# cvxopt/smcp

Measured on AMD Instinct MI355X. Metric: Newton KKT solves/sec, higher is better.
Workload: dtype f64; 1 GPU; synth50k nested block-arrow SDP n=50000, 8073 cliques, m=100; kktsolver=chol, n=50000, cliques=8073, m=100, blkval_doubles=2493568, update_doubles=10689536, parallelism=single

## Files before the change

### smcp_amd/csrc/capi.hip

```cpp
#include <hip/hip_runtime.h>
#include <memory>
#include <unordered_map>

#include <algorithm>
#include <chrono>
#include <cstdio>
#include <cstring>
#include <map>
#include <new>
#include <atomic>
#include <thread>
#include <type_traits>
#include <vector>

#include "../../include/smcp_amd.h"
#include "constraints.hpp"
#include "context.hpp"
#include "hostpar.hpp"
#include "switches.hpp"
#include "front_generic.hip"
#include "front_mfma.hip"
#include "front_large.hip"
#include "front_top.hip"
#include "front_inv.hip"
#include "front_n16.hip"
#include "front_downfam.hip"
#include "front_fam.hip"
#include "front_upfam.hip"
#include "front_fam2.hip"
#include "front_lfsp.hip"
#include "front_leafgram.hip"
#include "front_famt.hip"
#include "front_flow.hip"
#include "front_mrc.hip"
#include "front_edm.hip"
#include "front_psd.hip"
#include "front_trmm.hip"
#include "front_syr2k.hip"
#include "front_symm.hip"

using namespace smcp;

#define HIPCHK(x)                                                                        \
  do {                                                                                   \
    hipError_t e_ = (x);                                                                 \
    if (e_ != hipSuccess) {                                                              \
      fprintf(stderr, "smcp_amd: HIP error %s at %s:%d\n", hipGetErrorString(e_), __FILE__, __LINE__); \
      return SMCP_EHIP;                                                                  \
    }                                                                                    \
  } while (0)

namespace {

enum {
  KID_chol_level = 0, KID_llt_level, KID_pinv_level, KID_gather_level, KID_completion_all,
  KID_hess_up_level, KID_hess_down_level, KID_hess_down_inv_all, KID_hess_up_inv_level, KID_scale_an,
  KID_factor_yaa, KID_trsm_fwd_level, KID_trsm_bwd_level, KID_amap, KID_aadj, KID_scatter_constraints,
  KID_dense_potrf, KID_dense_potrs, KID_vec_axpby, KID_axpby, KID_reduce_cliques, KID_reduce_final,
  KID_hess_up_mfma, KID_hess_down_mfma, KID_chol_mfma, KID_pinv_mfma, KID_prep_lk,
  KID_hess_up_mfma_hbm, KID_hess_down_mfma_hbm, KID_chol_mfma_hbm, KID_pinv_mfma_hbm,
  KID_gram_partial, KID_gram_reduce, KID_hess_up_pad,
  KID_lf_assemble, KID_lf_clear_upd, KID_lf_up1, KID_lf_up2, KID_lf_up3, KID_lf_down1, KID_lf_down2, KID_lf_down3,
  KID_lf_pinv1, KID_lf_pinv2, KID_lf_diag, KID_lf_chol_panel, KID_lf_chol_trail, KID_lf_pack_upd,
  KID_lf_prep_s, KID_lf_prep_row, KID_lf_prep_k, KID_factor_yaa_lds,
  KID_factor_inverse, KID_hess_down_inv_mfma, KID_hess_down_inv_mfma_hbm, KID_hess_up_inv_mfma, KID_hess_up_inv_mfma_hbm,
  KID_completion_mfma, KID_completion_mfma_hbm, KID_lf_copy_an, KID_lf_ri_an, KID_lf_dinv1, KID_lf_dinv2,
  KID_lf_uinv1, KID_lf_uinv2, KID_lf_completion, KID_hess_up_n16, KID_llt_mfma, KID_llt_mfma_hbm, KID_lf_llt,
  KID_hess_up_fam, KID_qr_rmul, KID_qr_dots, KID_qr_comb, KID_qr_small, KID_fam2_prep, KID_mid_chol, KID_lf_diag_inv, KID_lfsp_up, KID_lfsp_prep, KID_leaf_gram, KID_leaf_tables, KID_fam_sparse, KID_gram_diag128, KID_lf_assemble_lds, KID_fam_terms, KID_famt_prep, KID_lf_assemble_lds_dyn, KID_lf_zsp, KID_fam_terms_grp, KID_lf_assemble_fz, KID_factor_inverse_lds, KID_chol_flow,
  KID_mrc_diag, KID_mrc_rank, KID_mrc_reduce, KID_mrc_factor, KID_cut_signs, KID_cut_weights,
  KID_edm_rank, KID_edm_reduce, KID_edm_factor, KID_edm_dense, KID_hess_down_fam, KID_hess_up_fam1,
  KID_psd_zero, KID_psd_scatter, KID_psd_solve, KID_psd_fill, KID_top_chol, KID_lf_trtri,
  KID_trmm_n, KID_trmm_t, KID_trmm_mm, KID_trmm_combine, KID_syr2k_fma, KID_syr2k_mm,
  KID_symm_fma, KID_symm_mm, KID_symm_combine,
  KID_potrs_many_small, KID_potrs_many_step, KID_aadj_sub_many, KID_kkt_many_y, KID_kkt_many_scale,
  KID_qr_dots_many, KID_qr_many_sum, KID_qr_many_small, KID_qr_many_mid, KID_qr_comb_many,
  KID_res_inv_table, KID_res_combine, KID_res_y, KID_res_norms, KID_kkt_many_sub,
  KID_COUNT
};
const char* const KID_NAMES[KID_COUNT] = {
  "k_chol_level", "k_llt_level", "k_pinv_level", "k_gather_level", "k_completion_all",
  "k_hess_up_level", "k_hess_down_level", "k_hess_down_inv_all", "k_hess_up_inv_level", "k_scale_an",
  "k_factor_yaa", "k_trsm_fwd_level", "k_trsm_bwd_level", "k_amap", "k_aadj", "k_scatter_constraints",
  "k_dense_potrf", "k_dense_potrs", "k_vec_axpby", "k_axpby", "k_reduce_cliques", "k_reduce_final",
  "k_hess_up_mfma<true>", "k_hess_down_mfma<true>", "k_chol_mfma<true>", "k_pinv_mfma<true>", "k_prep_lk",
  "k_hess_up_mfma<false>", "k_hess_down_mfma<false>", "k_chol_mfma<false>", "k_pinv_mfma<false>",
  "k_gram_partial", "k_gram_reduce", "k_hess_up_pad",
  "k_lf_assemble", "k_lf_clear_upd", "k_lf_up1", "k_lf_up2", "k_lf_up3", "k_lf_down1", "k_lf_down2", "k_lf_down3",
  "k_lf_pinv1", "k_lf_pinv2", "k_lf_diag", "k_lf_chol_panel", "k_lf_chol_trail", "k_lf_pack_upd",
  "k_lf_prep_s", "k_lf_prep_row", "k_lf_prep_k", "k_factor_yaa_lds",
  "k_factor_inverse", "k_hess_down_inv_mfma<true>", "k_hess_down_inv_mfma<false>", "k_hess_up_inv_mfma<true>",
  "k_hess_up_inv_mfma<false>", "k_completion_mfma<true>", "k_completion_mfma<false>", "k_lf_copy_an", "k_lf_ri_an",
  "k_lf_dinv1", "k_lf_dinv2", "k_lf_uinv1", "k_lf_uinv2", "k_lf_completion", "k_hess_up_n16",
  "k_llt_mfma<true>", "k_llt_mfma<false>", "k_lf_llt", "k_hess_up_fam",
  "k_stack_trsm", "k_stack_dots", "k_stack_comb", "k_qr_small", "k_fam2_prep", "k_mid_chol", "k_lf_diag_inv", "k_lfsp_up", "k_lfsp_prep", "k_leaf_pairs", "k_leaf_tables", "k_fam_sparse", "k_gram_diag128", "k_lf_assemble_lds", "k_fam_terms", "k_famt_prep", "k_lf_assemble_lds_dyn", "k_lf_zsp", "k_fam_terms_grp", "k_lf_assemble_fz", "k_factor_inverse_lds", "k_chol_flow",
  "k_mrc_diag", "k_mrc_rank", "k_mrc_reduce", "k_mrc_factor", "k_cut_signs", "k_cut_weights",
  "k_edm_rank", "k_edm_reduce", "k_edm_factor", "k_edm_dense", "k_hess_down_fam", "k_hess_up_fam1",
  "k_psd_zero", "k_psd_scatter", "k_psd_solve", "k_psd_fill", "k_top_chol", "k_lf_trtri",
  "k_trmm_n", "k_trmm_t", "k_trmm_mm", "k_trmm_combine", "k_syr2k_fma", "k_syr2k_mm",
  "k_symm_fma", "k_symm_mm", "k_symm_combine",
  "k_potrs_many_small", "k_potrs_many_step", "k_aadj_sub_many", "k_kkt_many_y", "k_kkt_many_scale",
  "k_stack_dots_many", "k_qr_many_sum", "k_qr_many_small", "k_qr_many_mid", "k_stack_comb_many",
  "k_res_inv_table", "k_res_combine", "k_res_y", "k_res_norms", "k_kkt_many_sub"};

inline void note_launch(csp_ctx* c, int kid) {
  const hipError_t e = hipGetLastError();
  if (e != hipSuccess && !c->launch_err) {
    c->launch_err = (int)e;
    fprintf(stderr, "smcp_amd: launch of %s failed: %s\n", (kid >= 0 && kid < KID_COUNT) ? KID_NAMES[kid] : "?", hipGetErrorString(e));
  }
}
inline hipError_t end_call(csp_ctx* c) {
  hipError_t e = hipGetLastError();
  if (e == hipSuccess && c->launch_err) e = c->launch_err > 0 ? (hipError_t)c->launch_err : hipErrorLaunchFailure;
  c->launch_err = 0;
  return e;
}

__global__ void k_race_spin(long long ticks) {
  const long long t0 = wall_clock64();
  for (int it = 0; it < (1 << 22) && wall_clock64() - t0 < ticks; ++it) __builtin_amdgcn_s_sleep(8);
}
struct RaceInject {
  std::atomic<uint64_t> state{0};
  std::atomic<int64_t> injected{0};
  std::atomic<int> max_us{200};
  std::atomic<int> drop_joins{0};
  bool on() const { return state.load(std::memory_order_relaxed) != 0; }
  void seed(uint64_t s) { state.store(s ? (s * 0x9E3779B97F4A7C15ull) | 1ull : 0ull); }
  uint64_t next() {
    uint64_t x = state.load(std::memory_order_relaxed);
    x ^= x << 13; x ^= x >> 7; x ^= x << 17;
    state.store(x | 1ull, std::memory_order_relaxed);
    return x;
  }
};
// ... 1725 lines not shown
      f.resize(S.nsn, 0);
      return put64(f);
    }
    case CSP_Q_MRC_CLAMPED:
      if (out) out[0] = c->mrc_clamped;
      return 1;
    case CSP_Q_EDM_CLAMPED:
      if (out) out[0] = c->edm_clamped;
      return 1;
  }
  return SMCP_EINVAL;
}

int csp_maxcardsearch(int64_t n, const int64_t* colptr, const int64_t* rowind, int64_t* order) {
  if (n <= 0 || !colptr || !rowind || !order) return SMCP_EINVAL;
  maxcardsearch(n, colptr, rowind, order);
  return 0;
}
int csp_mindegree(int64_t n, const int64_t* colptr, const int64_t* rowind, int64_t* order) {
  if (n <= 0 || !colptr || !rowind || !order) return SMCP_EINVAL;
  mindegree(n, colptr, rowind, order);
  return 0;
}
int csp_index_map(const csp_ctx* c, int64_t cnt, const int64_t* I, const int64_t* J, int64_t* out) {
  if (!c || cnt < 0) return SMCP_EINVAL;
  index_map(c->S, cnt, I, J, out);
  return 0;
}

}

#include "setup.hip"

extern "C" {

int64_t csp_device_bytes(const csp_ctx* c) { return c ? c->D.mem.total : 0; }

static int cholesky_impl(csp_ctx* c, double* x, void* stream, int set, bool li_last = false);
int csp_cholesky(csp_ctx* c, double* x, void* stream) { return cholesky_impl(c, x, stream, 0); }
int csp_cholesky_part(csp_ctx* c, double* x, int set, void* stream) {
  if (set < 1 || set > 2 || !c || !c->sets[set].lev2 || use_generic(c)) return SMCP_EINVAL;
  return cholesky_impl(c, x, stream, set);
}
static int cholesky_impl(csp_ctx* c, double* x, void* stream, int set, bool li_last) {
  if (int rc = ready(c)) return rc;
  invalidate_tags(c, x);
  hipStream_t st = (hipStream_t)stream;
  TreeArgs a = tree_args(c);
  HIPCHK(zero_flag(c, st));
  if (!use_generic(c)) {
    MfmaArgs a0 = mfma_args(c, nullptr, 0, 1);
    a0.LK = nullptr;
    for (int64_t l = 0; l < c->S.nlev; ++l)
      for_level_classes(c, l, a0, [&](bool lds, MfmaArgs am, int cnt, size_t bytes, int thr) {
        if (lds) launch_lds(c, KID_chol_mfma, k_chol_mfma<true>, dim3(cnt), dim3(fact_threads(am, thr, 0)),
                            (size_t)mfma_lds_doubles_for(WK_CHOL, am.nnmax, am.namax) * sizeof(double), st, am, x, (double*)nullptr);
        else if (use_large() && c->D.gp_tptr) lf_chol(c, am, cnt, x, st, li_last && l == c->S.nlev - 1);
        else launch_lds(c, KID_chol_mfma_hbm, k_chol_mfma<false>, dim3(cnt), dim3(thr), 0, st, am, x, (double*)nullptr);
      }, set);
  } else
  for_levels_up(c, [&](const int32_t* lev, int cnt) {
    a.lev = lev;
    launch(c, KID_chol_level, k_chol_level, dim3(cnt), dim3(NT), st, a, x);
  });
  HIPCHK(end_call(c));
  return fetch_info(c, st);
}

int csp_llt(csp_ctx* c, double* x, void* stream) {
  if (int rc = ready(c)) return rc;
  invalidate_tags(c, x);
  hipStream_t st = (hipStream_t)stream;
  TreeArgs a = tree_args(c);
  if (!use_generic(c)) {
    MfmaArgs a0 = mfma_args(c, nullptr, 0, 1);
    a0.LK = nullptr;
    dim3 blk(256);
    for (int64_t l = 0; l < c->S.nlev; ++l)
      for_level_classes(c, l, a0, [&](bool lds, MfmaArgs am, int cnt, size_t bytes, int thr) {
        if (lds) launch_lds(c, KID_llt_mfma, k_llt_mfma<true>, dim3(cnt), dim3(thr), bytes, st, am, x);
        else if (use_large()) {
          const int mtA = tiles64(am.namax), ntN = tiles64(am.nnmax);
          const int ntile = ntN * (ntN + 1) / 2 + mtA * ntN + mtA * (mtA + 1) / 2;
          launch(c, KID_lf_llt, k_lf_llt, dim3(umax1(ntile), cnt), blk, st, am, x, 0);
          launch(c, KID_lf_llt, k_lf_llt, dim3(umax1(ntile), cnt), blk, st, am, x, 1);
          lf_assemble(c, am, cnt, 1, x, 0, 2, st);
          if (am.namax) launch(c, KID_lf_pack_upd, k_lf_pack_upd, dim3(umax1(std::min(64, (am.namax * am.namax + 255) / 256)), cnt), blk, st, am);
        } else launch_lds(c, KID_llt_mfma_hbm, k_llt_mfma<false>, dim3(cnt), dim3(thr), 0, st, am, x);
      });
  } else
  for_levels_up(c, [&](const int32_t* lev, int cnt) {
    a.lev = lev;
    launch(c, KID_llt_level, k_llt_level, dim3(cnt), dim3(NT), st, a, x);
  });
  HIPCHK(end_call(c));
  return 0;
}

static int projected_inverse_impl(csp_ctx* c, double* x, void* stream, int set, bool have_li = false);
int csp_projected_inverse(csp_ctx* c, double* x, void* stream) { return projected_inverse_impl(c, x, stream, 0); }
int csp_projected_inverse_part(csp_ctx* c, double* x, int set, void* stream) {
  if (set < 1 || set > 2 || !c || !c->sets[set].lev2 || use_generic(c)) return SMCP_EINVAL;
  return projected_inverse_impl(c, x, stream, set);
}
static int projected_inverse_impl(csp_ctx* c, double* x, void* stream, int set, bool have_li) {
  if (int rc = ready(c)) return rc;
  invalidate_tags(c, x);
  hipStream_t st = (hipStream_t)stream;
  TreeArgs a = tree_args(c);
  if (!use_generic(c)) {
    if (set) { prep_lk_set(c, set, x, st); c->D.lk_tag_L = nullptr; c->D.lk_tag_Y = nullptr; }
    else {
    prep_lk(c, x, st, have_li);
    c->D.lk_tag_L = nullptr;
    c->D.lk_tag_Y = x;
    }
    const bool whole = !set;
    MfmaArgs a0 = mfma_args(c, nullptr, 0, 1);
    const bool keep_yaa = !set && !cache_off() && c->D.yaa && c->S.updlen() > 0;
    if (keep_yaa) a0.t.upd = c->D.yaa;
    for (int64_t l = c->S.nlev - 1; l >= 0; --l)
      for_level_classes(c, l, a0, [&](bool lds, MfmaArgs am, int cnt, size_t bytes, int thr) {
        if (lds) launch_lds(c, KID_pinv_mfma, k_pinv_mfma<true>, dim3(cnt), dim3(fact_threads(am, thr, 1)),
                            (size_t)mfma_lds_doubles_for(WK_PINV, am.nnmax, am.namax) * sizeof(double), st, am, x);
        else if (use_large()) lf_pinv(c, am, cnt, x, st);
        else launch_lds(c, KID_pinv_mfma_hbm, k_pinv_mfma<false>, dim3(cnt), dim3(thr), 0, st, am, x);
      }, set);
    if (keep_yaa) {
      c->D.yaa_tag = x;
      c->D.fac_tag = c->D.faci_tag = nullptr;
      c->D.part_valid = false;
      fp_record(c, 2, x, st);
    }
    if (whole) fp_record(c, 1, x, st);
  } else
  for_levels_down(c, [&](const int32_t* lev, int cnt) {
    a.lev = lev;
    launch(c, KID_pinv_level, k_pinv_level, dim3(cnt), dim3(NT), st, a, x);
  });
  HIPCHK(end_call(c));
  return 0;
}

constexpr int SCALING_FAC = 1;
static bool leafgram_ok(csp_ctx* c, int64_t mcols);
static bool scaling_overlap_on() {
  static int on = -1;
  if (on < 0) { const char* e = sw_str("SMCP_SCALING_OVERLAP"); on = (e && e[0] == '0') ? 0 : 1; }
  return on == 1;
}
static int scaling_impl(csp_ctx* c, double* L, double* Y, int flags, hipStream_t st) {
  DeviceCtx& D = c->D;
  const Symbolic& S = c->S;
  const int64_t bl = S.blklen();
  if (c->scal_lstar < 0) {
    int64_t ls = S.nlev;
    while (ls > 0 && c->lvl[(size_t)ls - 1].nI == 0) --ls;
    c->scal_lstar = ls;
    std::vector<int> lev_of((size_t)S.nsn, 0);
    for (int64_t l = 0; l < S.nlev; ++l)
      for (int64_t q = S.levptr[l]; q < S.levptr[l + 1]; ++q) lev_of[(size_t)S.levidx[q]] = (int)l;
    int64_t t0 = bl;
    for (int64_t k = 0; k < S.nsn; ++k) if (lev_of[(size_t)k] == S.nlev - 1) t0 = std::min<int64_t>(t0, S.blkptr[k]);
    for (int64_t k = 0; k < S.nsn; ++k) if (S.blkptr[k] >= t0 && lev_of[(size_t)k] != S.nlev - 1) { t0 = 0; break; }
    c->scal_tail0 = t0;
  }
  const int64_t lstar = c->scal_lstar;
  const bool fast = !use_generic(c) && use_large() && D.gp_tptr && !cache_off() && Fork::enabled() && scaling_overlap_on() &&
                    c->ntrial == 1 && lstar < S.nlev && (lstar > 0 || D.nI_total == 0) && D.yaa && S.updlen() > 0 && !c->verify_cache;
  if (!fast) {
    const bool li = top_li_whole(c);
    if (li) { D.lk_tag_L = D.lk_tag_Y = nullptr; D.part_valid = false; D.lk_gen++; }
    if (int rc = cholesky_impl(c, L, (void*)st, 0, li)) return rc;
    HIPCHK(hipMemcpyAsync(Y, L, sizeof(double) * bl, hipMemcpyDeviceToDevice, st));
    if (int rc = projected_inverse_impl(c, Y, (void*)st, 0, li)) return rc;
    c->D.lk_tag_L = L;
    if (flags & SCALING_FAC) { if (int rc = prepare_yaa(c, Y, true, st)) return rc; HIPCHK(end_call(c)); }
    return 0;
  }
  invalidate_tags(c, L);
  invalidate_tags(c, Y);
  HIPCHK(zero_flag(c, st));
  const int64_t last = S.nlev - 1;
  const int64_t tail0 = c->scal_tail0;
  MfmaArgs a0 = mfma_args(c, nullptr, 0, 1);
  a0.LK = nullptr;
  TreeArgs t = tree_args(c);
  int nnI = 0;
  for (const LevelClass& Lc : c->lvl) if (Lc.nI) nnI = std::max(nnI, (int)Lc.nnmaxI);
  static int cprep = -1;
  if (cprep < 0) { const char* e = sw_str("SMCP_CHOL_PREP"); cprep = (e && e[0] == '0') ? 0 : 1; }
  const bool fuse_prep = cprep && nnI <= 16;
  auto chol_level = [&](int64_t l) {
    for_level_classes(c, l, a0, [&](bool lds, MfmaArgs am, int cnt, size_t bytes, int thr) {
      (void)bytes;
      const size_t lb = (size_t)mfma_lds_doubles_for(WK_CHOL, am.nnmax, am.namax) * sizeof(double);
      if (lds && fuse_prep) launch_lds(c, KID_chol_mfma, k_chol_mfma<true, true>, dim3(cnt), dim3(fact_threads(am, thr, 0)), lb, st, am, L, D.lk);
      else if (lds) launch_lds(c, KID_chol_mfma, k_chol_mfma<true>, dim3(cnt), dim3(fact_threads(am, thr, 0)), lb, st, am, L, (double*)nullptr);
      else lf_chol(c, am, cnt, L, st, l == last);
    });
  };
  for (int64_t l = 0; l < last; ++l) chol_level(l);
  std::unique_ptr<Fork> f0;
  if (last > 0) f0.reset(new Fork(c, st, 1));
  hipStream_t s0 = f0 ? f0->s : st;
  chol_level(last);
  if (D.nI_total && !fuse_prep) {
    TreeArgs ts = t;
    ts.lev = D.lev3idx;
    launch_lds(c, KID_prep_lk, k_prep_lk, dim3((int)D.nI_total), dim3(prep_lk_threads(nnI)), prep_lk_lds_bytes(nnI), s0, ts, (const double*)L, D.lk);
  }
  for (int64_t ll = 0; ll < last; ++ll)
    for_level_classes(c, ll, a0, [&](bool lds, MfmaArgs am, int cnt, size_t, int) { if (!lds) lf_prep(c, am, cnt, L, s0); });
  if (tail0 > 0) (void)hipMemcpyAsync(Y, L, sizeof(double) * tail0, hipMemcpyDeviceToDevice, s0);
  for_level_classes(c, last, a0, [&](bool lds, MfmaArgs am, int cnt, size_t, int) { if (!lds) lf_prep(c, am, cnt, L, st, use_top(am.nnmax + am.namax)); });
  (void)hipMemcpyAsync(Y + tail0, L + tail0, sizeof(double) * (bl - tail0), hipMemcpyDeviceToDevice, st);
  if (f0) f0->join();
  D.lk_gen++;
  D.part_valid = false;
  MfmaArgs ap = mfma_args(c, nullptr, 0, 1);
  ap.t.upd = D.yaa;
  MfmaArgs af = mfma_args(c, nullptr, 0, 1);
  const bool want_fac = (flags & SCALING_FAC) != 0;
  static int skipenv = -1;
  if (skipenv < 0) { const char* e = sw_str("SMCP_FAC_PARTIAL"); skipenv = (e && e[0] == '0') ? 0 : 1; }
  const bool skip_children = want_fac && skipenv && D.m > 0 && !D.ns && leafgram_ok(c, D.m) && c->leafgram_policy != 0;
  bool skipped = false;
  auto factor_level = [&](int64_t l, hipStream_t lds_stream, hipStream_t large_stream) {
    for_level_classes(c, l, af, [&](bool lds, MfmaArgs am, int cnt, size_t, int) {
      if (!am.namax) return;
      if (lds) {
        if (l == 0 && skip_children && am.nS > 0) { cnt -= am.nS; skipped = true; if (!cnt) return; }
        const size_t bytes = ((size_t)padld(am.namax) * am.namax + 256 + 8) * sizeof(double);
        launch_lds(c, KID_factor_yaa_lds, k_factor_yaa_lds, dim3(cnt), dim3(fact_threads(am, 256, 2)), bytes, lds_stream, am, (const double*)D.yaa, D.fac);
      } else {
        launch(c, KID_axpby, k_copy_upd_blocks, dim3(cnt, umax1(std::min(64, (am.namax * am.namax + 1023) / 1024))), dim3(256), large_stream,
               am.t, (const double*)D.yaa, D.fac);
        lf_factor_yaa(c, am, cnt, D.fac, large_stream);
      }
    });
  };
  auto pinv_level = [&](int64_t l) {
    for_level_classes(c, l, ap, [&](bool lds, MfmaArgs am, int cnt, size_t bytes, int thr) {
      (void)bytes;
      if (lds) launch_lds(c, KID_pinv_mfma, k_pinv_mfma<true>, dim3(cnt), dim3(fact_threads(am, thr, 1)),
                          (size_t)mfma_lds_doubles_for(WK_PINV, am.nnmax, am.namax) * sizeof(double), st, am, Y);
      else lf_pinv(c, am, cnt, Y, st);
    });
  };
  for (int64_t l = last; l >= lstar; --l) pinv_level(l);
  bool any_large_sep = false;
  for (int64_t l = lstar; l <= last; ++l) if (c->lvl[(size_t)l].nII && c->lvl[(size_t)l].namaxII > 0) any_large_sep = true;
  std::unique_ptr<Fork> f1;
  if (want_fac && any_large_sep && lstar > 0) f1.reset(new Fork(c, st, 0));
  hipStream_t s1 = f1 ? f1->s : st;
  for (int64_t l = lstar - 1; l >= 0; --l) pinv_level(l);
  if (want_fac) {
    for (int64_t l = last; l >= lstar; --l) factor_level(l, s1, s1);
    for (int64_t l = lstar - 1; l >= 0; --l) factor_level(l, st, st);
  }
  if (f1) f1->join();
  D.lk_tag_L = L; D.lk_tag_Y = Y;
  D.yaa_tag = Y;
  D.fac_tag = want_fac ? Y : nullptr;
  D.fac_partial = want_fac && skipped;
  D.faci_tag = nullptr;
  if (want_fac) D.fac_gen++;
  HIPCHK(end_call(c));
  const int rc = fetch_info(c, st);
  if (rc) {
    D.lk_tag_L = D.lk_tag_Y = D.yaa_tag = D.fac_tag = D.faci_tag = nullptr;
    D.part_valid = false;
  }
  return rc;
}
int csp_cholesky_projected_inverse(csp_ctx* c, double* L, double* Y, int with_factors, void* stream) {
  if (int rc = ready(c)) return rc;
  if (!L || !Y || L == Y) return SMCP_EINVAL;
  return scaling_impl(c, L, Y, with_factors ? SCALING_FAC : 0, (hipStream_t)stream);
}

int csp_completion(csp_ctx* c, double* x, void* stream) {
  if (int rc = ready(c)) return rc;
  invalidate_tags(c, x);
  hipStream_t st = (hipStream_t)stream;
  TreeArgs a = tree_args(c);
  HIPCHK(zero_flag(c, st));
  if (!use_generic(c)) {
    prepare_yaa(c, x, true, st, true);
// ... 336 lines not shown
```

### smcp_amd/csrc/switches.hpp

```cpp
#pragma once
#include <cstdio>
#include <cstdlib>
#include <cstring>
#include <string>

extern char** environ;

namespace smcp {

struct Switch { const char* name; const char* dflt; const char* doc; };

static const Switch SWITCHES[] = {
  {"SMCP_GENERIC", "0", "1: any-size fixed-order kernels of front_generic.hip for every tree operation (as CSP_TUNE_DETERMINISTIC)"},
  {"SMCP_LARGE", "1", "0: no tiled large-front kernels (fronts beyond LDS take the one-workgroup HBM kernels)"},
  {"SMCP_NOCACHE", "0", "1: nothing derived from (L, Y) is reused between calls"},
  {"SMCP_FORK", "1", "0: no side streams, everything on the caller's stream"},
  {"SMCP_AUX_PRIO", "1", "0: side stream 0 (few-workgroup chains) at default instead of highest priority"},
  {"SMCP_AUX_PRIO1", "1", "0: side stream 1 (filler work) at default instead of lowest priority"},
  {"SMCP_EVENT_SYSFENCE", "0", "1: internal events with the default system-scope release (12 us per hand-over instead of 7)"},
  {"SMCP_SCALING_OVERLAP", "1", "0: csp_cholesky_projected_inverse as its three steps one after the other"},
  {"SMCP_CHOL_PREP", "1", "0: k_prep_lk in a launch of its own instead of inside k_chol_mfma (narrow supernodes)"},
  {"SMCP_FAC_PARTIAL", "1", "0: chol(Y_AA) of the family children always formed by the fused scaling point"},
  {"SMCP_MID", "1", "0: per-step kernels instead of k_mid_chol / k_lf_diag_inv for fronts of at most 272 rows"},
  {"SMCP_TOP_FUSED", "1", "0: k_mid_chol, and k_lf_diag_inv / k_lf_trtri for the inverse at the scaling point, instead of the register-resident k_top_chol for fronts of at most 208 rows"},
  {"SMCP_TRTRI", "1", "0: block-row triangular inversion of large fronts instead of recursive doubling"},
  {"SMCP_N16", "1", "0: no shape-specialised k_hess_up_n16"},
  {"SMCP_OLDLDS", "0", "1: k_hess_up_mfma<true> instead of the padded / n16 kernels"},
  {"SMCP_DOWN_W", "1", "0: k_hess_down_mfma instead of the one-wave k_hess_down_w"},
  {"SMCP_DOWN_FAM", "1", "most right-hand sides of a root -> leaves sweep that take the one-launch family kernel k_hess_down_fam (0: never; the per-level k_hess_down_w launches)"},
  {"SMCP_UP_FAM", "1", "most dense right-hand sides of a leaves -> root sweep that take the resident family kernel k_hess_up_fam1, the level-0 cliques outside the families riding along (0: never; k_hess_up_fam and a launch of their own for those cliques)"},
  {"SMCP_FAM", "1", "0: no family kernels (per-level sweeps with the update exchange through HBM)"},
  {"SMCP_FAM2", "1", "0: no sparse-input family kernels (k_fam_sparse, k_fam_terms): k_hess_up_fam"},
  {"SMCP_FAMT", "1", "0: no entry-driven family sweep k_fam_terms (k_fam_sparse instead)"},
  {"SMCP_FZ", "1", "0: the family parents' packed updates go through HBM (k_fam_terms writes, the extend-add reads) instead of being formed by k_lf_assemble_fz"},
  {"SMCP_FAMT_GROUP", "1", "0: no sibling groups of family parents (k_fam_terms_grp)"},
  {"SMCP_LFSP", "1", "0: dense phases instead of the sparse-input sweep k_lfsp_up of childless large fronts"},
  {"SMCP_LFSP_GROUP", "1", "0: no sibling groups in k_lfsp_up"},
  {"SMCP_ZSP", "1", "0: dense first phase of wide childless fronts instead of k_lf_zsp"},
  {"SMCP_LEAFGRAM", "1", "0: never the closed-form Gram blocks of the family children (k_leaf_tables / k_leaf_pairs)"},
  {"SMCP_LG_SIDE", "1", "0: leaf Gram blocks after the sweep on the caller's stream instead of beside the top phases"},
  {"SMCP_GRAM_EARLY", "0", "1: the Gram chunks of the levels 0 / 1 rows on the side branch beside the top fronts' phase kernels (measured slower: 3.37 against 3.22 ms per step)"},
  {"SMCP_LG_EARLY", "1", "0: leaf Gram blocks beside the phase kernels of the top fronts instead of from the start of the sweep"},
  {"SMCP_FACI_LDS", "1", "0: inverse Y_AA factors of the small fronts by block rows against HBM (k_factor_inverse) instead of in LDS"},
  {"SMCP_FZ_TAIL", "1", "0: every (front, right-hand side) pair of the fused extend-add is one workgroup's task, also in a thin last round"},
  {"SMCP_GRAM", "1", "0: reference (two-sweep) formulation of the Schur complement instead of the Gram formulation"},
  {"SMCP_SCM", "1", "0: column-sparse constraints swept like the others (no SCMcolumn2 route)"},
  {"SMCP_TRSM_MM", "1", "0: csp_trsm through the generic level kernels instead of tile products"},
  {"SMCP_TRMM_MM", "1", "0: no MFMA tile products in csp_trmm (every front on the FMA kernels); 2: tile products for the large fronts only, also from 32 columns on"},
  {"SMCP_SYR2K_MM", "1", "0: no MFMA tile products in csp_syr2k (every front on the FMA kernel); 2: tile products for the large fronts only, whatever the rank (read on every call)"},
  {"SMCP_SYMM_MM", "1", "0: no MFMA tile products in csp_symm (every front on the FMA kernel); 2: tile products for the large fronts only, whatever the column count (read on every call)"},
  {"SMCP_POTRS_MANY_MM", "1", "0: no MFMA tile products in the block steps of dense_potrs_many / kkt_solve_many (FMA updates whatever the column count; read on every call)"},
  {"SMCP_ALDS", "1", "0: extend-add of large fronts by gather plan only (no LDS streaming kernel)"},
  {"SMCP_ALDS_DYN", "1", "0: one workgroup per (front, right-hand side) instead of the task-drawing grid"},
  {"SMCP_ALDS_FILL", "1", "0: k_panel_fill builds the input panels instead of the extend-add (sgn 3)"},
  {"SMCP_ASM", "plan", "t: tiled extend-add kernel instead of the gather plan"},
  {"SMCP_ROOT_FUSED", "0", "1: fused two-product sweep of fronts without separator (Y_NN explicit: condition squared; studies only)"},
  {"SMCP_PD", "0", "1: four-wave tile products everywhere (no sixteen-wave shape for small launches)"},
  {"SMCP_FLOW", "1", "0: no one-launch blocked Cholesky with in-launch tile dataflow (front_flow.hip): per-step kernels for dense matrices / single fronts beyond 272 rows"},
  {"SMCP_FLOW_WG", "112", "workgroups of that launch (at most 112: four launches fit the chip side by side)"},
  {"SMCP_POTRF_DEFER", "1", "0: kkt_schur_factor factors H at once even under deferred status"},
  {"SMCP_QR_TRSM", "mfma", "f: vector-FMA substitution kernel of kkt_qr instead of the MFMA one"},
  {"SMCP_FTHR_CHOL", "128", "threads of k_chol_mfma on the leaf class"},
  {"SMCP_FTHR_PINV", "256", "threads of k_pinv_mfma on the leaf class"},
// ... 64 lines not shown
```

Before: 341.8 KKT solves/s.

## Fuse level-0/1 family Cholesky and projected-inverse sweeps into single LDS-resident kernels

Adds k_chol_fam and k_pinv_fam. Each runs a whole level-1 parent together with its level-0 children in one workgroup, and it can also take the lone level-0 cliques. The children's update matrices are extend-added through LDS atomics, where before they took per-level launches with an HBM round trip. The fused kernels are used in the plain Cholesky, the projected inverse and the scaling-point paths when the tree has only small fronts below level 2. The goal is to cut launch count and HBM traffic for the many tiny cliques, at the cost of a lot of new specialised code and LDS-atomic accumulation order.

```diff
diff --git a/smcp_amd/csrc/capi.hip b/smcp_amd/csrc/capi.hip
--- a/smcp_amd/csrc/capi.hip
+++ b/smcp_amd/csrc/capi.hip
@@ -27,6 +27,8 @@
 #include "front_downfam.hip"
 #include "front_fam.hip"
 #include "front_upfam.hip"
+#include "front_cholfam.hip"
+#include "front_pinvfam.hip"
 #include "front_fam2.hip"
 #include "front_lfsp.hip"
 #include "front_leafgram.hip"
@@ -75,6 +77,7 @@
   KID_potrs_many_small, KID_potrs_many_step, KID_aadj_sub_many, KID_kkt_many_y, KID_kkt_many_scale,
   KID_qr_dots_many, KID_qr_many_sum, KID_qr_many_small, KID_qr_many_mid, KID_qr_comb_many,
   KID_res_inv_table, KID_res_combine, KID_res_y, KID_res_norms, KID_kkt_many_sub,
+  KID_chol_fam, KID_pinv_fam,
   KID_COUNT
 };
 const char* const KID_NAMES[KID_COUNT] = {
@@ -100,7 +103,8 @@
   "k_symm_fma", "k_symm_mm", "k_symm_combine",
   "k_potrs_many_small", "k_potrs_many_step", "k_aadj_sub_many", "k_kkt_many_y", "k_kkt_many_scale",
   "k_stack_dots_many", "k_qr_many_sum", "k_qr_many_small", "k_qr_many_mid", "k_stack_comb_many",
-  "k_res_inv_table", "k_res_combine", "k_res_y", "k_res_norms", "k_kkt_many_sub"};
+  "k_res_inv_table", "k_res_combine", "k_res_y", "k_res_norms", "k_kkt_many_sub",
+  "k_chol_fam", "k_pinv_fam"};
 
 inline void note_launch(csp_ctx* c, int kid) {
   const hipError_t e = hipGetLastError();
@@ -1892,6 +1896,102 @@
 
 #include "setup.hip"
 
+namespace {
+
+struct ScalFam {
+  bool on = false;
+  MfmaArgs af;
+  int nfam = 0;
+  const int32_t* lone = nullptr;
+  int nlone = 0, lnn = 0, lna = 0;
+  int nfmax = 0, cpan = 0, sel = 0;
+  size_t bytes = 0;
+};
+ScalFam scaling_fam_plan(csp_ctx* c, const MfmaArgs& a0, int set) {
+  ScalFam p;
+  static const int on = sw_on("SMCP_SCALING_FAM", 1);
+  if (!on || set || use_generic(c) || fam_off() || c->verify_cache || c->ntrial != 1 || c->sets[1].lev2 || c->sets[2].lev2 || c->S.nlev < 2) return p;
+  const LevelClass& L0 = c->lvl[0];
+  const LevelClass& L1 = c->lvl[1];
+  if (!L1.nI || !L1.nS || !L0.nS) return p;
+  for (int64_t l = 2; l < c->S.nlev; ++l) if (c->lvl[(size_t)l].nS) return p;
+  if (L1.famnn > 16 || L1.famna > 64 || L1.famcnn > 16 || L1.famcna > 32) return p;
+  p.af = a0;
+  p.af.t.lev = c->D.lev2idx + c->S.levptr[1] + (L1.nI - L1.nS);
+  p.af.level = 1;
+  p.af.famna = L1.famna; p.af.famnn = L1.famnn; p.af.famcna = L1.famcna; p.af.famcnn = L1.famcnn;
+  p.nfam = (int)L1.nS;
+  const int nout = (int)(L0.nI - L0.nS);
+  if (nout > 0 && L0.nnmaxI <= 16 && L0.namaxI <= 64) { p.lone = c->D.lev2idx + c->S.levptr[0]; p.nlone = nout; p.lnn = L0.nnmaxI; p.lna = L0.namaxI; }
+  p.nfmax = std::max(L1.famnn + L1.famna, p.lnn + p.lna);
+  p.cpan = (L1.famcnn + L1.famcna) * L1.famcnn;
+  p.bytes = sfam_lds_bytes(p.nfmax, p.cpan);
+  if (p.bytes > 64 * 1024) return p;
+  const int pnat = (std::max(std::max((int)L1.famna, p.lna), 1) + 15) / 16, cnat = (std::max((int)L1.famcna, 1) + 15) / 16;
+  p.sel = 2 * pnat + cnat;
+  p.on = p.sel >= 3 && p.sel <= 10;
+  return p;
+}
+template <bool PREP>
+bool launch_chol_fam(csp_ctx* c, const ScalFam& p, double* x, double* lkout, hipStream_t st) {
+  const dim3 grid(p.nfam + p.nlone), blk(256);
+#define SMCP_CF(PN, CN) launch_lds(c, KID_chol_fam, k_chol_fam<PN, CN, PREP>, grid, blk, p.bytes, st, p.af, x, lkout, p.nfmax, p.cpan, p.nfam, p.lone); return true
+  switch (p.sel) {
+    case 3: SMCP_CF(1, 1);
+    case 4: SMCP_CF(1, 2);
+    case 5: SMCP_CF(2, 1);
+    case 6: SMCP_CF(2, 2);
+    case 7: SMCP_CF(3, 1);
+    case 8: SMCP_CF(3, 2);
+    case 9: SMCP_CF(4, 1);
+    case 10: SMCP_CF(4, 2);
+  }
+#undef SMCP_CF
+  return false;
+}
+bool launch_pinv_fam(csp_ctx* c, const ScalFam& p, const MfmaArgs& ap, double* x, hipStream_t st) {
+  MfmaArgs af = p.af;
+  af.t.upd = ap.t.upd; af.LK = ap.LK;
+  const dim3 grid(p.nfam + p.nlone), blk(256);
+#define SMCP_PF(PN, CN) launch_lds(c, KID_pinv_fam, k_pinv_fam<PN, CN>, grid, blk, p.bytes, st, af, x, p.nfmax, p.cpan, p.nfam, p.lone); return true
+  switch (p.sel) {
+    case 3: SMCP_PF(1, 1);
+    case 4: SMCP_PF(1, 2);
+    case 5: SMCP_PF(2, 1);
+    case 6: SMCP_PF(2, 2);
+    case 7: SMCP_PF(3, 1);
+    case 8: SMCP_PF(3, 2);
+    case 9: SMCP_PF(4, 1);
+    case 10: SMCP_PF(4, 2);
+  }
+#undef SMCP_PF
+  return false;
+}
+template <class Small, class Large, class Fam>
+void scaling_fam_up(csp_ctx* c, const ScalFam& p, const MfmaArgs& a0, Small small, Large large, Fam fam) {
+  for (int64_t l = 0; l < 2; ++l) {
+    if (l == 1) fam();
+    for_level_classes(c, l, a0, [&](bool lds, MfmaArgs am, int cnt, size_t, int thr) {
+      if (!lds) { large(am, cnt, l); return; }
+      cnt -= am.nS;
+      if (cnt > 0 && !(l == 0 && p.nlone)) small(am, cnt, thr);
+    });
+  }
+}
+template <class Small, class Large, class Fam>
+void scaling_fam_down(csp_ctx* c, const ScalFam& p, const MfmaArgs& a0, Small small, Large large, Fam fam) {
+  for (int64_t l = 1; l >= 0; --l) {
+    if (l == 0) fam();
+    for_level_classes(c, l, a0, [&](bool lds, MfmaArgs am, int cnt, size_t, int thr) {
+      if (!lds) { large(am, cnt, l); return; }
+      cnt -= am.nS;
+      if (cnt > 0 && !(l == 0 && p.nlone)) small(am, cnt, thr);
+    });
+  }
+}
+
+}
+
 extern "C" {
 
 int64_t csp_device_bytes(const csp_ctx* c) { return c ? c->D.mem.total : 0; }
@@ -1911,12 +2011,21 @@
   if (!use_generic(c)) {
     MfmaArgs a0 = mfma_args(c, nullptr, 0, 1);
     a0.LK = nullptr;
-    for (int64_t l = 0; l < c->S.nlev; ++l)
+    auto small = [&](const MfmaArgs& am, int cnt, int thr) {
+      launch_lds(c, KID_chol_mfma, k_chol_mfma<true>, dim3(cnt), dim3(fact_threads(am, thr, 0)),
+                 (size_t)mfma_lds_doubles_for(WK_CHOL, am.nnmax, am.namax) * sizeof(double), st, am, x, (double*)nullptr);
+    };
+    auto large = [&](const MfmaArgs& am, int cnt, int64_t l) {
+      if (use_large() && c->D.gp_tptr) lf_chol(c, am, cnt, x, st, li_last && l == c->S.nlev - 1);
+      else launch_lds(c, KID_chol_mfma_hbm, k_chol_mfma<false>, dim3(cnt), dim3(1024), 0, st, am, x, (double*)nullptr);
+    };
+    const ScalFam sf = scaling_fam_plan(c, a0, set);
+    if (sf.on) scaling_fam_up(c, sf, a0, small, large, [&]() { launch_chol_fam<false>(c, sf, x, (double*)nullptr, st); });
+    for (int64_t l = sf.on ? 2 : 0; l < c->S.nlev; ++l)
       for_level_classes(c, l, a0, [&](bool lds, MfmaArgs am, int cnt, size_t bytes, int thr) {
-        if (lds) launch_lds(c, KID_chol_mfma, k_chol_mfma<true>, dim3(cnt), dim3(fact_threads(am, thr, 0)),
-                            (size_t)mfma_lds_doubles_for(WK_CHOL, am.nnmax, am.namax) * sizeof(double), st, am, x, (double*)nullptr);
-        else if (use_large() && c->D.gp_tptr) lf_chol(c, am, cnt, x, st, li_last && l == c->S.nlev - 1);
-        else launch_lds(c, KID_chol_mfma_hbm, k_chol_mfma<false>, dim3(cnt), dim3(thr), 0, st, am, x, (double*)nullptr);
+        (void)bytes;
+        if (lds) small(am, cnt, thr);
+        else large(am, cnt, l);
       }, set);
   } else
   for_levels_up(c, [&](const int32_t* lev, int cnt) {
@@ -1979,13 +2088,22 @@
     MfmaArgs a0 = mfma_args(c, nullptr, 0, 1);
     const bool keep_yaa = !set && !cache_off() && c->D.yaa && c->S.updlen() > 0;
     if (keep_yaa) a0.t.upd = c->D.yaa;
-    for (int64_t l = c->S.nlev - 1; l >= 0; --l)
+    auto small = [&](const MfmaArgs& am, int cnt, int thr) {
+      launch_lds(c, KID_pinv_mfma, k_pinv_mfma<true>, dim3(cnt), dim3(fact_threads(am, thr, 1)),
+                 (size_t)mfma_lds_doubles_for(WK_PINV, am.nnmax, am.namax) * sizeof(double), st, am, x);
+    };
+    auto large = [&](const MfmaArgs& am, int cnt, int64_t) {
+      if (use_large()) lf_pinv(c, am, cnt, x, st);
+      else launch_lds(c, KID_pinv_mfma_hbm, k_pinv_mfma<false>, dim3(cnt), dim3(1024), 0, st, am, x);
+    };
+    const ScalFam sf = scaling_fam_plan(c, a0, set);
+    for (int64_t l = c->S.nlev - 1; l >= (sf.on ? 2 : 0); --l)
       for_level_classes(c, l, a0, [&](bool lds, MfmaArgs am, int cnt, size_t bytes, int thr) {
-        if (lds) launch_lds(c, KID_pinv_mfma, k_pinv_mfma<true>, dim3(cnt), dim3(fact_threads(am, thr, 1)),
-                            (size_t)mfma_lds_doubles_for(WK_PINV, am.nnmax, am.namax) * sizeof(double), st, am, x);
-        else if (use_large()) lf_pinv(c, am, cnt, x, st);
-        else launch_lds(c, KID_pinv_mfma_hbm, k_pinv_mfma<false>, dim3(cnt), dim3(thr), 0, st, am, x);
+        (void)bytes;
+        if (lds) small(am, cnt, thr);
+        else large(am, cnt, l);
       }, set);
+    if (sf.on) scaling_fam_down(c, sf, a0, small, large, [&]() { launch_pinv_fam(c, sf, a0, x, st); });
     if (keep_yaa) {
       c->D.yaa_tag = x;
       c->D.fac_tag = c->D.faci_tag = nullptr;
@@ -2051,16 +2169,26 @@
   static int cprep = -1;
   if (cprep < 0) { const char* e = sw_str("SMCP_CHOL_PREP"); cprep = (e && e[0] == '0') ? 0 : 1; }
   const bool fuse_prep = cprep && nnI <= 16;
+  auto chol_small = [&](const MfmaArgs& am, int cnt, int thr) {
+    const size_t lb = (size_t)mfma_lds_doubles_for(WK_CHOL, am.nnmax, am.namax) * sizeof(double);
+    if (fuse_prep) launch_lds(c, KID_chol_mfma, k_chol_mfma<true, true>, dim3(cnt), dim3(fact_threads(am, thr, 0)), lb, st, am, L, D.lk);
+    else launch_lds(c, KID_chol_mfma, k_chol_mfma<true>, dim3(cnt), dim3(fact_threads(am, thr, 0)), lb, st, am, L, (double*)nullptr);
+  };
+  auto chol_large = [&](const MfmaArgs& am, int cnt, int64_t l) { lf_chol(c, am, cnt, L, st, l == last); };
   auto chol_level = [&](int64_t l) {
     for_level_classes(c, l, a0, [&](bool lds, MfmaArgs am, int cnt, size_t bytes, int thr) {
       (void)bytes;
-      const size_t lb = (size_t)mfma_lds_doubles_for(WK_CHOL, am.nnmax, am.namax) * sizeof(double);
-      if (lds && fuse_prep) launch_lds(c, KID_chol_mfma, k_chol_mfma<true, true>, dim3(cnt), dim3(fact_threads(am, thr, 0)), lb, st, am, L, D.lk);
-      else if (lds) launch_lds(c, KID_chol_mfma, k_chol_mfma<true>, dim3(cnt), dim3(fact_threads(am, thr, 0)), lb, st, am, L, (double*)nullptr);
-      else lf_chol(c, am, cnt, L, st, l == last);
+      if (lds) chol_small(am, cnt, thr);
+      else chol_large(am, cnt, l);
     });
   };
-  for (int64_t l = 0; l < last; ++l) chol_level(l);
+  const ScalFam sf = scaling_fam_plan(c, a0, 0);
+  if (sf.on)
+    scaling_fam_up(c, sf, a0, chol_small, chol_large, [&]() {
+      if (fuse_prep) launch_chol_fam<true>(c, sf, L, D.lk, st);
+      else launch_chol_fam<false>(c, sf, L, (double*)nullptr, st);
+    });
+  for (int64_t l = sf.on ? 2 : 0; l < last; ++l) chol_level(l);
   std::unique_ptr<Fork> f0;
   if (last > 0) f0.reset(new Fork(c, st, 1));
   hipStream_t s0 = f0 ? f0->s : st;
@@ -2100,12 +2228,16 @@
       }
     });
   };
+  auto pinv_small = [&](const MfmaArgs& am, int cnt, int thr) {
+    launch_lds(c, KID_pinv_mfma, k_pinv_mfma<true>, dim3(cnt), dim3(fact_threads(am, thr, 1)),
+               (size_t)mfma_lds_doubles_for(WK_PINV, am.nnmax, am.namax) * sizeof(double), st, am, Y);
+  };
+  auto pinv_large = [&](const MfmaArgs& am, int cnt, int64_t) { lf_pinv(c, am, cnt, Y, st); };
   auto pinv_level = [&](int64_t l) {
     for_level_classes(c, l, ap, [&](bool lds, MfmaArgs am, int cnt, size_t bytes, int thr) {
       (void)bytes;
-      if (lds) launch_lds(c, KID_pinv_mfma, k_pinv_mfma<true>, dim3(cnt), dim3(fact_threads(am, thr, 1)),
-                          (size_t)mfma_lds_doubles_for(WK_PINV, am.nnmax, am.namax) * sizeof(double), st, am, Y);
-      else lf_pinv(c, am, cnt, Y, st);
+      if (lds) pinv_small(am, cnt, thr);
+      else pinv_large(am, cnt, l);
     });
   };
   for (int64_t l = last; l >= lstar; --l) pinv_level(l);
@@ -2114,7 +2246,8 @@
   std::unique_ptr<Fork> f1;
   if (want_fac && any_large_sep && lstar > 0) f1.reset(new Fork(c, st, 0));
   hipStream_t s1 = f1 ? f1->s : st;
-  for (int64_t l = lstar - 1; l >= 0; --l) pinv_level(l);
+  for (int64_t l = lstar - 1; l >= (sf.on ? 2 : 0); --l) pinv_level(l);
+  if (sf.on) scaling_fam_down(c, sf, ap, pinv_small, pinv_large, [&]() { launch_pinv_fam(c, sf, ap, Y, st); });
   if (want_fac) {
     for (int64_t l = last; l >= lstar; --l) factor_level(l, s1, s1);
     for (int64_t l = lstar - 1; l >= 0; --l) factor_level(l, st, st);
diff --git a/smcp_amd/csrc/front_cholfam.hip b/smcp_amd/csrc/front_cholfam.hip
--- /dev/null
+++ b/smcp_amd/csrc/front_cholfam.hip
@@ -0,0 +1,264 @@
+#include <hip/hip_runtime.h>
+
+namespace smcp {
+
+__host__ __device__ inline int sfam_wave_doubles(int cpan) { return cpan + 256 + 16; }
+__host__ inline size_t sfam_lds_bytes(int nfmax, int cpan) { return (size_t)(nfmax * (nfmax + 1) / 2 + 2 + 4 * sfam_wave_doubles(cpan)) * sizeof(double); }
+struct SfamStage { double* P; double* D; int32_t* rel; };
+__device__ inline SfamStage sfam_stage_of(double* zs, int nfmax, int wave, int cpan) {
+  double* w = zs + nfmax * (nfmax + 1) / 2 + 2 + (size_t)wave * sfam_wave_doubles(cpan);
+  return SfamStage{w, w + cpan, (int32_t*)(w + cpan + 256)};
+}
+__device__ inline void sfam_stage(const SfamStage& st, const double* src, int pan, int lane) {
+  for (int e0 = 0; e0 < pan; e0 += 256) {
+    double v[4];
+#pragma unroll
+    for (int h = 0; h < 4; ++h) {
+      const int e = e0 + 64 * h + lane;
+      v[h] = e < pan ? src[(unsigned)e] : 0.0;
+    }
+#pragma unroll
+    for (int h = 0; h < 4; ++h) {
+      const int e = e0 + 64 * h + lane;
+      if (e < pan) st.P[e] = v[h];
+    }
+  }
+}
+__device__ inline void sfam_stage_rel(const SfamStage& st, const TreeArgs& t, const CliqueDesc& d, int lane) {
+  if (lane < d.na) st.rel[lane] = t.relidx[d.rel + lane];
+}
+struct SfamPre { double v[4]; int rel; };
+__device__ inline void sfam_fetch(SfamPre& p, const double* src, int pan, const TreeArgs& t, const CliqueDesc& d, int lane) {
+#pragma unroll
+  for (int h = 0; h < 4; ++h) {
+    const int e = 64 * h + lane;
+    p.v[h] = e < pan ? src[(unsigned)e] : 0.0;
+  }
+  p.rel = lane < d.na ? t.relidx[d.rel + lane] : 0;
+}
+__device__ inline void sfam_commit(const SfamStage& st, const SfamPre& p, int pan, const CliqueDesc& d, int lane) {
+#pragma unroll
+  for (int h = 0; h < 4; ++h) {
+    const int e = 64 * h + lane;
+    if (e < pan) st.P[e] = p.v[h];
+  }
+  if (lane < d.na) st.rel[lane] = p.rel;
+}
+
+template <int NATC, bool PREP>
+__device__ inline bool chol_fam_child(const SfamStage& st, const CliqueDesc& cd, double* Pc, double* lkc, double* zs, int nfz, int lane) {
+  const int l15 = lane & 15, kq = lane >> 4;
+  const int nnc = cd.nn, nac = cd.na, nfc = nnc + nac;
+  const int ksnc = (nnc + 3) >> 2;
+  const d4 zero4 = {0.0, 0.0, 0.0, 0.0};
+  wave_sync();
+  const bool ok = wave_potrf_inv16(st.P, nfc, nnc, st.D);
+  if (!ok) return false;
+  wave_sync();
+  double lir[4], lic[4], san[NATC][4];
+  int rm[NATC];
+#pragma unroll
+  for (int s = 0; s < 4; ++s) {
+    const int kk = kq + 4 * s;
+    lir[s] = (l15 < nnc && kk <= l15) ? st.D[l15 + kk * 16] : 0.0;
+    lic[s] = (kk < nnc && l15 <= kk) ? st.D[kk + l15 * 16] : 0.0;
+    if (l15 < nnc && kk <= l15) Pc[l15 + kk * nfc] = st.P[l15 + kk * nfc];
+    if (PREP && l15 < nnc && kk < nnc) lkc[l15 + kk * nfc] = lir[s];
+#pragma unroll
+    for (int t = 0; t < NATC; ++t) {
+      const int m = 16 * t + l15;
+      san[t][s] = (m < nac && kk < nnc) ? st.P[nnc + m + kk * nfc] : 0.0;
+    }
+  }
+#pragma unroll
+  for (int t = 0; t < NATC; ++t) {
+    const int m = 16 * t + l15;
+    rm[t] = m < nac ? st.rel[m] : -1;
+  }
+  d4 accL[NATC];
+#pragma unroll
+  for (int t = 0; t < NATC; ++t) {
+    accL[t] = zero4;
+    if (16 * t >= nac) continue;
+#pragma unroll
+    for (int s = 0; s < 4; ++s)
+      if (s < ksnc) fmma(accL[t], san[t][s], lir[s]);
+    d4 accK = zero4;
+    if (PREP) {
+#pragma unroll
+      for (int s = 0; s < 4; ++s)
+        if (s < ksnc) fmma(accK, accL[t][s], lic[s]);
+    }
+#pragma unroll
+    for (int rr = 0; rr < 4; ++rr) {
+      const int m = 16 * t + l15, n = kq + 4 * rr;
+      if (m < nac && n < nnc) {
+        Pc[(nnc + m) + n * nfc] = accL[t][rr];
+        if (PREP) lkc[(nnc + m) + n * nfc] = accK[rr];
+      }
+    }
+  }
+#pragma unroll
+  for (int tm = 0; tm < NATC; ++tm)
+#pragma unroll
+    for (int tn = 0; tn <= tm; ++tn) {
+      if (16 * tm >= nac) continue;
+      d4 acc = zero4;
+#pragma unroll
+      for (int s = 0; s < 4; ++s)
+        if (s < ksnc) fmma(acc, accL[tm][s], accL[tn][s]);
+      const int ri = rm[tm];
+#pragma unroll
+      for (int rr = 0; rr < 4; ++rr) {
+        const int n = 16 * tn + kq + 4 * rr;
+        if (ri >= 0 && n < nac && 16 * tm + l15 >= n) unsafeAtomicAdd(&zs[pk_low(ri, st.rel[n], nfz)], -acc[rr]);
+      }
+    }
+  wave_sync();
+  return true;
+}
+
+template <int PNAT, int CNAT, bool PREP>
+__global__ void __launch_bounds__(256, 4) k_chol_fam(MfmaArgs a, double* x, double* lkout, int nfmax, int cpan, int nfam, const int32_t* lone) {
+  extern __shared__ double zs[];
+  const int tid = threadIdx.x;
+  const int lane = tid & 63, l15 = lane & 15, kq = lane >> 4;
+  const int wave = __builtin_amdgcn_readfirstlane((int)(threadIdx.x >> 6));
+  const int k = (int)blockIdx.x < nfam ? a.t.lev[blockIdx.x] : lone[(int)blockIdx.x - nfam];
+  const CliqueDesc d = a.t.cl[k];
+  const int nn = d.nn, na = d.na, nf = nn + na;
+  const int nch = (int)blockIdx.x < nfam ? d.chend - d.chbeg : 0;
+  int* const sflag = (int*)(zs + nfmax * (nfmax + 1) / 2);
+  if (tid == 0) {
+    sflag[0] = *info_of(a.t, k); sflag[1] = 0; sflag[2] = 0;
+    if (nch > 8) { atomicCAS(info_of(a.t, k), 0, -7); sflag[0] = 1; }
+  }
+  double* const P = x + d.blk;
+  double* const UkP = a.t.updp + d.updp;
+  const int ksn = (nn + 3) >> 2;
+  const d4 zero4 = {0.0, 0.0, 0.0, 0.0};
+  const bool has0 = wave < nch, has1 = wave + 4 < nch;
+  const int kc0 = has0 ? a.t.chidx[d.chbeg + wave] : k, kc1 = has1 ? a.t.chidx[d.chbeg + wave + 4] : k;
+  const CliqueDesc dc0 = a.t.cl[kc0];
+  const CliqueDesc dc1 = a.t.cl[kc1];
+  const SfamStage st = sfam_stage_of(zs, nfmax, wave, cpan);
+  if (has0) { sfam_stage(st, x + dc0.blk, (dc0.nn + dc0.na) * dc0.nn, lane); sfam_stage_rel(st, a.t, dc0, lane); }
+  {
+    double v[8];
+#pragma unroll
+    for (int c = 0; c < 4; ++c) {
+      const int j = wave + 4 * c;
+#pragma unroll
+      for (int h = 0; h < 2; ++h) {
+        const int i = j + lane + 64 * h;
+        v[2 * c + h] = (j < nn && i < nf) ? P[i + j * nf] : 0.0;
+      }
+    }
+#pragma unroll
+    for (int c = 0; c < 4; ++c) {
+      const int j = wave + 4 * c;
+#pragma unroll
+      for (int h = 0; h < 2; ++h) {
+        const int i = j + lane + 64 * h;
+        if (j < nn && i < nf) zs[pk_low(i, j, nf)] = v[2 * c + h];
+      }
+    }
+    for (int e = pk_low(nn, nn, nf) + tid; e < nf * (nf + 1) / 2; e += 256) zs[e] = 0.0;
+  }
+  __syncthreads();
+  if (sflag[0]) return;
+  if (has0) {
+    const int pan1 = (dc1.nn + dc1.na) * dc1.nn;
+    const bool pre1 = has1 && pan1 <= 256;
+    SfamPre pre;
+    if (pre1) sfam_fetch(pre, x + dc1.blk, pan1, a.t, dc1, lane);
+    bool ok = chol_fam_child<CNAT, PREP>(st, dc0, x + dc0.blk, lkout + dc0.blk, zs, nf, lane);
+    int kf = kc0;
+    if (ok && has1) {
+      if (pre1) sfam_commit(st, pre, pan1, dc1, lane);
+      else { sfam_stage(st, x + dc1.blk, pan1, lane); sfam_stage_rel(st, a.t, dc1, lane); }
+      ok = chol_fam_child<CNAT, PREP>(st, dc1, x + dc1.blk, lkout + dc1.blk, zs, nf, lane);
+      kf = kc1;
+    }
+    if (!ok && lane == 0) { atomicCAS(info_of(a.t, kf), 0, info_val(a.t, kf)); sflag[1] = 1; }
+  }
+  __syncthreads();
+  if (sflag[1]) return;
+  double* const Sd = sfam_stage_of(zs, nfmax, 1, cpan).D;
+  double* const Dv = sfam_stage_of(zs, nfmax, 0, cpan).D;
+  if (wave == 0) {
+#pragma unroll
+    for (int r = 0; r < 4; ++r) {
+      const int c = kq + 4 * r;
+      if (l15 < nn && c <= l15) Sd[l15 + c * 16] = zs[pk_low(l15, c, nf)];
+    }
+    wave_sync();
+    const bool ok = wave_potrf_inv16(Sd, 16, nn, Dv);
+    if (!ok) { if (lane == 0) { atomicCAS(info_of(a.t, k), 0, info_val(a.t, k)); sflag[2] = 1; } }
+    else {
+      wave_sync();
+#pragma unroll
+      for (int r = 0; r < 4; ++r) {
+        const int c = kq + 4 * r;
+        if (l15 < nn && c <= l15) P[l15 + c * nf] = Sd[l15 + c * 16];
+        if (PREP && l15 < nn && c < nn) (lkout + d.blk)[l15 + c * nf] = c <= l15 ? Dv[l15 + c * 16] : 0.0;
+      }
+    }
+  }
+  __syncthreads();
+  if (sflag[2]) return;
+  const int gw = wave;
+  if (gw >= PNAT || 16 * gw >= na) return;
+  double lir[4], lic[4];
+#pragma unroll
+  for (int s = 0; s < 4; ++s) {
+    const int kk = kq + 4 * s;
+    lir[s] = (l15 < nn && kk <= l15) ? Dv[l15 + kk * 16] : 0.0;
+    lic[s] = (kk < nn && l15 <= kk) ? Dv[kk + l15 * 16] : 0.0;
+  }
+  d4 accL[PNAT];
+#pragma unroll
+  for (int t = 0; t < PNAT; ++t) {
+    accL[t] = zero4;
+    if (t > gw) continue;
+    const int m = 16 * t + l15;
+    double san[4];
+#pragma unroll
+    for (int s = 0; s < 4; ++s) san[s] = (m < na && kq + 4 * s < nn) ? zs[pk_low(nn + m, kq + 4 * s, nf)] : 0.0;
+#pragma unroll
+    for (int s = 0; s < 4; ++s)
+      if (s < ksn) fmma(accL[t], san[s], lir[s]);
+  }
+  d4 accM = zero4, accK = zero4;
+#pragma unroll
+  for (int t = 0; t < PNAT; ++t) if (t == gw) accM = accL[t];
+  if (PREP) {
+#pragma unroll
+    for (int s = 0; s < 4; ++s)
+      if (s < ksn) fmma(accK, accM[s], lic[s]);
+  }
+  const int m = 16 * gw + l15;
+#pragma unroll
+  for (int rr = 0; rr < 4; ++rr) {
+    const int n = kq + 4 * rr;
+    if (m < na && n < nn) {
+      P[(nn + m) + n * nf] = accM[rr];
+      if (PREP) (lkout + d.blk)[(nn + m) + n * nf] = accK[rr];
+    }
+  }
+#pragma unroll
+  for (int tn = 0; tn < PNAT; ++tn) {
+    if (tn > gw) continue;
+    d4 acc = zero4;
+#pragma unroll
+    for (int s = 0; s < 4; ++s)
+      if (s < ksn) fmma(acc, accM[s], accL[tn][s]);
+#pragma unroll
+    for (int rr = 0; rr < 4; ++rr) {
+      const int n = 16 * tn + kq + 4 * rr;
+      if (m >= n && m < na) UkP[n * na - ((n * (n - 1)) >> 1) + (m - n)] = zs[pk_low(nn + m, nn + n, nf)] - acc[rr];
+    }
+  }
+}
+
+}
diff --git a/smcp_amd/csrc/front_pinvfam.hip b/smcp_amd/csrc/front_pinvfam.hip
--- /dev/null
+++ b/smcp_amd/csrc/front_pinvfam.hip
@@ -0,0 +1,150 @@
+#include <hip/hip_runtime.h>
+
+namespace smcp {
+
+template <int NAT, bool OWN, int M>
+__device__ inline d4 pinv_fam_tiles(const double (&li)[4], const double (&kk)[4 * M], const CliqueDesc& d, double* P, double* yaa,
+                                    double* zs, int nfz, const int32_t* rel, int t0, int t1, bool with_li, int lane) {
+  const int l15 = lane & 15, kq = lane >> 4;
+  const int nn = d.nn, na = d.na, nf = nn + na;
+  const int ksn = (nn + 3) >> 2, ksa = (na + 3) >> 2;
+  const d4 zero4 = {0.0, 0.0, 0.0, 0.0};
+  d4 accN = zero4;
+  if (with_li) {
+#pragma unroll
+    for (int s = 0; s < 4; ++s)
+      if (s < ksn) fmma(accN, li[s], li[s]);
+  }
+#pragma unroll
+  for (int t = 0; t < NAT; ++t) {
+    if (t < t0 || t >= t1 || 16 * t >= na) continue;
+    const int m = 16 * t + l15;
+    int ri = 0;
+    if (!OWN) ri = rel[min(m, na - 1)];
+    d4 accE = zero4;
+#pragma unroll
+    for (int s0 = 0; s0 < 4 * NAT; s0 += 8) {
+      double y[8];
+#pragma unroll
+      for (int s = s0; s < s0 + 8 && s < 4 * NAT; ++s) {
+        const int j = kq + 4 * s;
+        const int i1 = OWN ? nn + min(m, na - 1) : ri, j1 = OWN ? nn + min(j, na - 1) : rel[min(j, na - 1)];
+        const double v = zs[pk_low(max(i1, j1), min(i1, j1), nfz)];
+        y[s - s0] = (m < na && j < na) ? v : 0.0;
+        if (!OWN && m < na && j <= m) yaa[m + j * na] = v;
+      }
+#pragma unroll
+      for (int s = s0; s < s0 + 8 && s < 4 * NAT; ++s)
+        if (s < ksa) fmma(accE, kk[s], y[s - s0]);
+    }
+#pragma unroll
+    for (int rr = 0; rr < 4; ++rr) {
+      const int mm = 16 * t + kq + 4 * rr;
+      if (mm < na && l15 < nn) {
+        P[nn + mm + l15 * nf] = -accE[rr];
+        if (OWN) zs[pk_low(nn + mm, l15, nfz)] = -accE[rr];
+      }
+    }
+#pragma unroll
+    for (int s = 0; s < 4; ++s) fmma(accN, kk[4 * t + s], accE[s]);
+  }
+  return accN;
+}
+
+template <int PNAT, int CNAT>
+__global__ void __launch_bounds__(256, 4) k_pinv_fam(MfmaArgs a, double* x, int nfmax, int cpan, int nfam, const int32_t* lone) {
+  extern __shared__ double zs[];
+  const int tid = threadIdx.x;
+  const int lane = tid & 63, l15 = lane & 15, kq = lane >> 4;
+  const int wave = __builtin_amdgcn_readfirstlane((int)(threadIdx.x >> 6));
+  const int k = (int)blockIdx.x < nfam ? a.t.lev[blockIdx.x] : lone[(int)blockIdx.x - nfam];
+  const CliqueDesc d = a.t.cl[k];
+  const int nn = d.nn, na = d.na, nf = nn + na;
+  const int nch = (int)blockIdx.x < nfam ? d.chend - d.chbeg : 0;
+  double* const P = x + d.blk;
+  const bool has0 = wave < nch, has1 = wave + 4 < nch;
+  const CliqueDesc dc0 = a.t.cl[has0 ? a.t.chidx[d.chbeg + wave] : k];
+  const CliqueDesc dc1 = a.t.cl[has1 ? a.t.chidx[d.chbeg + wave + 4] : k];
+  const SfamStage st = sfam_stage_of(zs, nfmax, wave, cpan);
+  if (has0) { sfam_stage(st, a.LK + dc0.blk, (dc0.nn + dc0.na) * dc0.nn, lane); sfam_stage_rel(st, a.t, dc0, lane); }
+  constexpr int M = PNAT > CNAT ? PNAT : CNAT;
+  double li[4], kk[4 * M];
+  down_fam_load_lk<PNAT, M>(li, kk, a.LK + d.blk, d, lane);
+  if (na > 0) {
+    const bool haspar = d.parent >= 0;
+    const CliqueDesc par = a.t.cl[haspar ? d.parent : k];
+    const int nng = par.nn, nag = par.na, nfg = nng + nag;
+    const double* Pg = x + par.blk;
+    const double* Ug = a.t.upd + par.upd;
+    double* const UkG = a.t.upd + d.upd;
+    const int32_t* rel = a.t.relidx + d.rel;
+    const int gi = rel[min(lane, na - 1)];
+    double v[4 * PNAT];
+#pragma unroll
+    for (int c = 0; c < 4 * PNAT; ++c) {
+      const int j = wave + 4 * c;
+      v[c] = 0.0;
+      if (haspar && j < na && lane >= j && lane < na) {
+        const int gj = rel[j];
+        const int hi = max(gi, gj), lo = min(gi, gj);
+        v[c] = lo < nng ? Pg[hi + (int64_t)lo * nfg] : Ug[(hi - nng) + (int64_t)(lo - nng) * nag];
+      }
+    }
+#pragma unroll
+    for (int c = 0; c < 4 * PNAT; ++c) {
+      const int j = wave + 4 * c;
+      if (j < na && lane >= j && lane < na) {
+        zs[pk_low(nn + lane, nn + j, nf)] = v[c];
+        if (haspar) UkG[lane + j * na] = v[c];
+      }
+    }
+  }
+  __syncthreads();
+  {
+    const d4 accN = pinv_fam_tiles<PNAT, true, M>(li, kk, d, P, nullptr, zs, nf, nullptr, wave, wave + 1, wave == 0, lane);
+#pragma unroll
+    for (int rr = 0; rr < 4; ++rr) st.D[l15 + 16 * (kq + 4 * rr)] = accN[rr];
+  }
+  __syncthreads();
+  {
+    const int i = tid & 15, j = tid >> 4;
+    if (i < nn && j <= i) {
+      double v = sfam_stage_of(zs, nfmax, 0, cpan).D[tid];
+#pragma unroll
+      for (int w = 1; w < 4; ++w)
+        if (w < PNAT && 16 * w < na) v += sfam_stage_of(zs, nfmax, w, cpan).D[tid];
+      zs[pk_low(i, j, nf)] = v;
+      P[i + j * nf] = v;
+    }
+  }
+  if (nch == 0) return;
+  __syncthreads();
+  const int pan1 = (dc1.nn + dc1.na) * dc1.nn;
+  const bool pre1 = has1 && pan1 <= 256;
+  SfamPre pre;
+  if (has0) {
+    down_fam_load_lk<CNAT, M>(li, kk, st.P, dc0, lane);
+    if (pre1) sfam_fetch(pre, a.LK + dc1.blk, pan1, a.t, dc1, lane);
+  }
+  auto child = [&](const CliqueDesc& dc) {
+    double* const Pc = x + dc.blk;
+    const d4 accN = pinv_fam_tiles<CNAT, false, M>(li, kk, dc, Pc, a.t.upd + dc.upd, zs, nf, st.rel, 0, CNAT, true, lane);
+    const int nfc = dc.nn + dc.na;
+#pragma unroll
+    for (int rr = 0; rr < 4; ++rr) {
+      const int c = kq + 4 * rr;
+      if (l15 < dc.nn && c <= l15) Pc[l15 + c * nfc] = accN[rr];
+    }
+  };
+  if (has0) child(dc0);
+  if (has1) {
+    wave_sync();
+    if (pre1) sfam_commit(st, pre, pan1, dc1, lane);
+    else { sfam_stage(st, a.LK + dc1.blk, pan1, lane); sfam_stage_rel(st, a.t, dc1, lane); }
+    wave_sync();
+    down_fam_load_lk<CNAT, M>(li, kk, st.P, dc1, lane);
+    child(dc1);
+  }
+}
+
+}
diff --git a/smcp_amd/csrc/switches.hpp b/smcp_amd/csrc/switches.hpp
--- a/smcp_amd/csrc/switches.hpp
+++ b/smcp_amd/csrc/switches.hpp
@@ -29,6 +29,7 @@
   {"SMCP_DOWN_W", "1", "0: k_hess_down_mfma instead of the one-wave k_hess_down_w"},
   {"SMCP_DOWN_FAM", "1", "most right-hand sides of a root -> leaves sweep that take the one-launch family kernel k_hess_down_fam (0: never; the per-level k_hess_down_w launches)"},
   {"SMCP_UP_FAM", "1", "most dense right-hand sides of a leaves -> root sweep that take the resident family kernel k_hess_up_fam1, the level-0 cliques outside the families riding along (0: never; k_hess_up_fam and a launch of their own for those cliques)"},
+  {"SMCP_SCALING_FAM", "1", "0: per-level k_chol_mfma / k_pinv_mfma launches for the families of the scaling point instead of one k_chol_fam / k_pinv_fam launch each way"},
   {"SMCP_FAM", "1", "0: no family kernels (per-level sweeps with the update exchange through HBM)"},
   {"SMCP_FAM2", "1", "0: no sparse-input family kernels (k_fam_sparse, k_fam_terms): k_hess_up_fam"},
   {"SMCP_FAMT", "1", "0: no entry-driven family sweep k_fam_terms (k_fam_sparse instead)"},
```

Result: faster. 354.9 KKT solves/s, median of 6 (+3.8%).
